# royshil/SfM-Toy-Library

Hardware: AMD Instinct MI355X
Metric: BA LM iterations/sec (200 cams, 100k pts, 1M obs) (higher is better)
Workload: dtype f32 Jacobian blocks and observation coordinates; a lane's own partial sum (<= 8 pair products of a block, ceil(track / 4) point-block products of a point) in f32, every sum across lanes, chunks, points and ranks in f64; residuals, cost, reduced system and solve in f64; 1 GPU; cfg3: 200 cams / 100000 pts / 1000000 obs, shared focal, two-level block-Jacobi PCG, one independent problem per GPU; step=one full LM solve to ceres CONVERGENCE from the resident initial point, linear_solver=two-level block-Jacobi PCG, tolerance 1e-08 anchored to the first LM iteration

## Files before the change

sfm-toy-library_amd/csrc/ba_common.h:

```cpp
#pragma once
#include "ba_kernels.h"
#include "sfmba_device.h"
#include "../../include/sfmba.h"

namespace sfmba {

#define BLK 256

__device__ inline void make_cam_table(const double cam[6], const double* scale6, double* ct) {
    const double w0 = cam[0], w1 = cam[1], w2 = cam[2];
    const double theta2 = w0 * w0 + w1 * w1 + w2 * w2;
    double R[9], K[9];
    double small = 0.0;
    double cq = 1.0 / 12.0;
    if (theta2 > DBL_EPSILON) {
        const double theta = sqrt(theta2);
        double s, c;
        sincos(theta, &s, &c);
        if (theta2 > 1e-8) { const double den = 2.0 * theta * s; cq = fabs(den) > 1e-12 ? 1.0 / theta2 - (1.0 + c) / den : 0.0; }
        const double ti = 1.0 / theta;
        const double k0 = w0 * ti, k1 = w1 * ti, k2 = w2 * ti;
        const double oc = 1.0 - c;
        R[0] = c + k0 * k0 * oc;       R[1] = k0 * k1 * oc - k2 * s;  R[2] = k0 * k2 * oc + k1 * s;
        R[3] = k0 * k1 * oc + k2 * s;  R[4] = c + k1 * k1 * oc;       R[5] = k1 * k2 * oc - k0 * s;
// ... 166 lines not shown
        HalvingReduceT<V, H, OFF / 2, VALU64>::run(v, lane, base, len);
    }
};
template <typename V, int N, bool VALU64>
struct HalvingReduceT<V, N, 0, VALU64> {
    static __device__ __forceinline__ void run(V*, int, int&, int&) {}
};
template <int N, int OFF> using HalvingReduce = HalvingReduceT<double, N, OFF>;

template <typename T>
__device__ __forceinline__ void load_obs(const void* base, int q, double& ox, double& oy) {
    const typename ObsXY<T>::type v = reinterpret_cast<const typename ObsXY<T>::type*>(base)[q];
    ox = (double)v.x; oy = (double)v.y;
}

#ifndef PBK
#define PBK 128
#endif
#define WPB (PBK / 64)

__device__ __forceinline__ void wave_lds_fence() {
    __builtin_amdgcn_fence(__ATOMIC_ACQ_REL, "workgroup");
    __builtin_amdgcn_wave_barrier();
}

#define PB_LPP 4

#define CD_N 48
#define CD_BLK 256
#define CD_OBS (SFMBA_CAM_CHUNK / CD_BLK)
// ... 100 lines not shown
```

sfm-toy-library_amd/csrc/ba_kernels.h:

```cpp
#pragma once
#include <hip/hip_runtime.h>
#include <vector>
#include <stdint.h>

#ifndef SFMBA_CAM_CHUNK
#define SFMBA_CAM_CHUNK 256
#endif

#ifndef SFMBA_PAIR_CHUNK
#define SFMBA_PAIR_CHUNK 512
#endif

namespace sfmba {

enum {
    ACC_TRIAL_COST = 0,
    ACC_MODEL = 1,
    ACC_STEP2 = 2,
    ACC_XNEW2 = 3,
    ACC_BAD_TRIAL = 4,
    ACC_GMAX = 5,
    ACC_BAD_LIN = 6,
    ACC_LIN_COST = 7,
    ACC_COUNT = 8,
// ... 107 lines not shown
    double* pcg_zero;
    int pcg_zero_n;
    double* pcg_bt;
    double* pcg_binv;
    double* pair_partial;
    double* pair_G;
    double* pcg_W;
    int* lm_mailbox;
    double* probe_z;
    double* probe_dpt;
    double shared_weight;
    float* shard_blocks32;
    double* shard_blocks;
    const double* shard_scal;
    const int* shard_row_shift;
};

template <typename T> void launch_cam_setup(hipStream_t s, const DeviceStructure& ds, const DeviceBuffers& db, int which);
void launch_begin(hipStream_t s, const DeviceStructure& ds, const DeviceBuffers& db, const LMState& st, const double* cam_src = nullptr,
                  const double* pts_src = nullptr);
void launch_xnorm(hipStream_t s, const DeviceStructure& ds, const DeviceBuffers& db);
template <typename T> void launch_colnorm(hipStream_t s, const DeviceStructure& ds, const DeviceBuffers& db, int jacobi_scaling, bool clear_udiag = true,
                                         bool points = true, bool finish_xnorm = false, bool with_xnorm = false);
void launch_colnorm_points_only(hipStream_t s, const DeviceStructure& ds, const DeviceBuffers& db, int jacobi, int precision_f32);
void launch_colnorm_cams_only(hipStream_t s, const DeviceStructure& ds, const DeviceBuffers& db, int jacobi, int precision_f32, bool clear_udiag = true);
void launch_colnorm_finish(hipStream_t s, const DeviceStructure& ds, const DeviceBuffers& db, int jacobi);
void launch_iter0(hipStream_t s, const DeviceStructure& ds, const DeviceBuffers& db);

template <typename T> void launch_point_build(hipStream_t s, const DeviceStructure& ds, const DeviceBuffers& db,
                                             int ps_mode = 0 );

template <typename T> void launch_cam_diag(hipStream_t s, const DeviceStructure& ds, const DeviceBuffers& db);

void launch_finalize(hipStream_t s, const DeviceStructure& ds, const DeviceBuffers& db, int pcg);
void launch_cd_fold(hipStream_t s, const DeviceStructure& ds, const DeviceBuffers& db);
void launch_gauge(hipStream_t s, const DeviceStructure& ds, const DeviceBuffers& db);

template <typename T> void launch_schur_pairs(hipStream_t s, const DeviceStructure& ds, const DeviceBuffers& db, int mode);

void launch_cam_update(hipStream_t s, const DeviceStructure& ds, const DeviceBuffers& db);
template <typename T> void launch_point_update(hipStream_t s, const DeviceStructure& ds, const DeviceBuffers& db);
void launch_control(hipStream_t s, const DeviceStructure& ds, const DeviceBuffers& db);

template <typename T> void launch_eval_residuals(hipStream_t s, const DeviceStructure& ds, const DeviceBuffers& db,
                                                 const int* perm, double* res_out, double* cost_out);
template <typename T> void launch_eval_jacobian(hipStream_t s, const DeviceStructure& ds, const DeviceBuffers& db,
                                                const int* obs_pt, const int* perm, double* jc, double* jp, double* jf);
void launch_mirror_scale(hipStream_t s, const DeviceStructure& ds, const DeviceBuffers& db, double* S_full, double* scale_out);

struct ImplicitProduct {
    DeviceStructure ds;
    DeviceBuffers db;
    double* dtab = nullptr;
    double* spt = nullptr;
    double* acc = nullptr;
    double* part = nullptr;
// ... 60 lines not shown
```

sfm-toy-library_amd/csrc/ba_points.hip:

```cpp
#include "ba_common.h"
#include <algorithm>

namespace sfmba {

__device__ __forceinline__ bool chol3_inverse(const double V[6] , double Li[6]) {
    const double i00 = fast_rsq(V[0]);
    const double l10 = V[1] * i00, l20 = V[3] * i00;
    const double d1 = V[2] - l10 * l10;
    const double i11 = fast_rsq(d1);
    const double l21 = (V[4] - l20 * l10) * i11;
    const double d2 = V[5] - l20 * l20 - l21 * l21;
    const double i22 = fast_rsq(d2);
    Li[0] = i00;
    Li[1] = -l10 * i00 * i11;
    Li[2] = i11;
    Li[4] = -l21 * i11 * i22;
    Li[3] = -(l20 * i00 + l21 * Li[1]) * i22;
    Li[5] = i22;
    return (V[0] > 0.0) && (d1 > 0.0) && (d2 > 0.0);
}

template <typename T>
__device__ __forceinline__ void point_finish(const DeviceBuffers& db, const LMState* st, size_t i, int ps_mode, const double (&Xl)[3], double (&V)[6], double (&bp)[3],
                                             double (&Ef)[3], double (&sp)[3], bool store, double& gmax, double& sff, double& rhsf, double& bad) {
// ... 34 lines not shown
    ra.X[0] = Xl[0]; ra.X[1] = Xl[1]; ra.X[2] = Xl[2];
    ra.L[0] = (T)(Li[0] * sp[0]); ra.L[1] = (T)(Li[1] * sp[0]); ra.L[2] = (T)(Li[2] * sp[1]);
    ra.L[3] = (T)(Li[3] * sp[0]); ra.L[4] = (T)(Li[4] * sp[1]); ra.L[5] = (T)(Li[5] * sp[2]);
    if (sizeof(T) == 8) reinterpret_cast<double*>(&ra)[9] = 0.0;
    reinterpret_cast<PtRecA<T>*>(db.PA)[i] = ra;
    PtRecB<T> rb;
    rb.t[0] = (T)t0; rb.t[1] = (T)t1; rb.t[2] = (T)t2;
    rb.yf[0] = (T)y0; rb.yf[1] = (T)y1; rb.yf[2] = (T)y2;
    reinterpret_cast<PtRecB<T>*>(db.PB)[i] = rb;
}

template <typename T>
__global__ __launch_bounds__(PBK) void k_point_build(DeviceStructure ds, DeviceBuffers db, int ps_mode_flags) {
    if ((ps_mode_flags & 4) && (db.st->termination != -1 || db.st->retry != 0)) return;
    const int ps_mode = ps_mode_flags & 3;
    __shared__ double scratch[WPB * 4];
    const LMState* st = db.st;
    const int cur = st->cur;
    const double* tab = db.camtab[cur];
    const double focal = st->focal[cur];
    const T fscale = (T)st->fscale;
    const double* pts = db.pts[cur];
    const int lane = threadIdx.x & 63, w = threadIdx.x >> 6;
    const int gw = blockIdx.x * WPB + w;
    double lin_cost = 0.0, sff = 0.0, rhsf = 0.0, gmax = 0.0, bad = 0.0;
    for (int e = blockIdx.x * blockDim.x + threadIdx.x; e < ds.ncam * 60; e += gridDim.x * blockDim.x) {
        const int j = e / 60, k = e - 60 * j, row0 = 6 * j;
        if (k < 36) db.S[(size_t)(row0 + k / 6) * ds.ld + row0 + k % 6] = 0.0;
        else if (k < 42) db.udiag[row0 + k - 36] = 0.0;
        else if (k < 48) db.bc[row0 + k - 42] = 0.0;
        else if (k < 54) db.rhs[row0 + k - 48] = 0.0;
        else db.S[(size_t)(row0 + k - 54) * ds.ld + ds.d - 1] = 0.0;
    }
    const int sub = lane & (PB_LPP - 1);
    const int slot = gw * (64 / PB_LPP) + (lane / PB_LPP);
    const bool have = slot < ds.npt;
    const int ip = have ? (ds.pt_order ? ds.pt_order[slot] : slot) : 0;
    const size_t i = (size_t)ip;
    const int q0 = have ? ds.pt_ptr[ip] : 0, q1 = have ? ds.pt_ptr[ip + 1] : 0;
    double Xl[3] = { pts[3 * i], pts[3 * i + 1], pts[3 * i + 2] };
    double sp[3] = { 1.0, 1.0, 1.0 };
    if (ps_mode == 0) { sp[0] = db.pscale[3 * i]; sp[1] = db.pscale[3 * i + 1]; sp[2] = db.pscale[3 * i + 2]; }
    T Va[6] = { (T)0, (T)0, (T)0, (T)0, (T)0, (T)0 }, Ea[3] = { (T)0, (T)0, (T)0 };
    double bp[3] = { 0, 0, 0 };
    int q = q0 + sub;
    int j_next = q < q1 ? ds.obs_cam[q] : 0;
    double ox_next = 0.0, oy_next = 0.0;
    if (q < q1) load_obs<T>(ds.obs_xy, q, ox_next, oy_next);
    while (__any(q < q1)) {
        const bool act = q < q1;
        const int j = j_next;
        const double ox = ox_next, oy = oy_next;
        const CamRow ct = { tab + 4 * (size_t)(j), ds.ncam };
        double Rt[12];
#pragma unroll
        for (int e = 0; e < 12; ++e) Rt[e] = ct[CT_R + e];
        q += PB_LPP;
        if (q < q1) { j_next = ds.obs_cam[q]; load_obs<T>(ds.obs_xy, q, ox_next, oy_next); }
        if (act) {
            const Proj pr = project_point(Rt, 0, 9, Xl);
            const double r0 = focal * pr.xp - ox, r1 = focal * pr.yp - oy;
            lin_cost += r0 * r0 + r1 * r1;
            T B[6];
            point_block<T>(Rt, pr, focal, B);
            const T g0 = (T)pr.xp * fscale, g1 = (T)pr.yp * fscale;
            Va[0] += B[0] * B[0] + B[3] * B[3];
            Va[1] += B[1] * B[0] + B[4] * B[3];
            Va[2] += B[1] * B[1] + B[4] * B[4];
            Va[3] += B[2] * B[0] + B[5] * B[3];
            Va[4] += B[2] * B[1] + B[5] * B[4];
            Va[5] += B[2] * B[2] + B[5] * B[5];
#pragma unroll
            for (int c = 0; c < 3; ++c) {
                Ea[c] += B[c] * g0 + B[3 + c] * g1;
                bp[c] += (double)B[c] * r0 + (double)B[3 + c] * r1;
            }
        }
    }
    double V[6], Ef[3];
#pragma unroll
    for (int c = 0; c < 6; ++c) { double v = (double)Va[c]; v = xlane_add<1>(v); v = xlane_add<2>(v); V[c] = v; }
#pragma unroll
    for (int c = 0; c < 3; ++c) {
        double v = (double)Ea[c]; v = xlane_add<1>(v); v = xlane_add<2>(v); Ef[c] = v;
        double u = bp[c]; u = xlane_add<1>(u); u = xlane_add<2>(u); bp[c] = u;
    }
    if (have) point_finish<T>(db, st, i, ps_mode, Xl, V, bp, Ef, sp, sub == 0, gmax, sff, rhsf, bad);
    if (!finite_d(lin_cost)) bad = 1.0;
    const double gm = wave_max(gmax);
    if ((threadIdx.x & 63) == 0 && gm > 0.0) atomic_max_nonneg(slot_ptr(db, ACC_GMAX), gm);
    double sums[4] = { lin_cost, sff, rhsf, bad };
    const double tot = block_sums<4>(sums, scratch);
    if (threadIdx.x < 4) {
        const int which = threadIdx.x == 0 ? ACC_LIN_COST : threadIdx.x == 1 ? ACC_SFF : threadIdx.x == 2 ? ACC_RHSF : ACC_BAD_LIN;
        if (threadIdx.x < 3 || tot != 0.0) atomicAdd(slot_ptr(db, which), tot);
    }
}

template <typename T>
void launch_point_build(hipStream_t s, const DeviceStructure& ds, const DeviceBuffers& db, int ps_mode) {
    const int per_wg = WPB * (64 / PB_LPP);
    hipLaunchKernelGGL(k_point_build<T>, dim3(std::max(1, (ds.npt + per_wg - 1) / per_wg)), dim3(PBK), 0, s, ds, db, ps_mode);
}
template void launch_point_build<float>(hipStream_t, const DeviceStructure&, const DeviceBuffers&, int);
template void launch_point_build<double>(hipStream_t, const DeviceStructure&, const DeviceBuffers&, int);

}
```

sfm-toy-library_amd/csrc/ba_setup.hip:

```cpp
#include "ba_common.h"
#include <algorithm>

namespace sfmba {

__global__ void k_cam_setup(int ncam, const double* __restrict__ cam, const double* __restrict__ cscale, double* __restrict__ camtab) {
    const int j = blockIdx.x * blockDim.x + threadIdx.x;
    if (j >= ncam) return;
    double c6[6], ct[CT_STRIDE];
    for (int e = 0; e < 6; ++e) c6[e] = cam[6 * j + e];
    make_cam_table(c6, cscale + 6 * j, ct);
    for (int e = 0; e < CT_STRIDE; ++e) camtab[cam_tab_index(e, j, ncam)] = ct[e];
}

template <typename T>
void launch_cam_setup(hipStream_t s, const DeviceStructure& ds, const DeviceBuffers& db, int which) {
    hipLaunchKernelGGL(k_cam_setup, dim3((ds.ncam + 63) / 64), dim3(64), 0, s, ds.ncam, db.cam[which], db.cscale, db.camtab[which]);
}
template void launch_cam_setup<float>(hipStream_t, const DeviceStructure&, const DeviceBuffers&, int);
template void launch_cam_setup<double>(hipStream_t, const DeviceStructure&, const DeviceBuffers&, int);

__global__ void k_begin(LMState st, DeviceStructure ds, DeviceBuffers db, const double* __restrict__ cam_src, const double* __restrict__ pts_src) {
    const int e = blockIdx.x * blockDim.x + threadIdx.x;
    if (e == 0) { *db.st = st; *db.lin_info = 0; *db.fin_counter = 0; }
    if (e < 6 * ds.ncam) db.cscale[e] = 1.0;
// ... 36 lines not shown
    hipLaunchKernelGGL(k_xnorm, dim3(blocks), dim3(BLK), 0, s, ds, db);
}

template <typename T>
__global__ __launch_bounds__(BLK) void k_colnorm_points(DeviceStructure ds, DeviceBuffers db, int jacobi) {
    const int i = blockIdx.x * blockDim.x + threadIdx.x;
    if (i >= ds.npt) return;
    const int cur = db.st->cur;
    const double* tab = db.camtab[cur];
    const double focal = db.st->focal[cur];
    const double X[3] = { db.pts[cur][3 * i], db.pts[cur][3 * i + 1], db.pts[cur][3 * i + 2] };
    double n0 = 0, n1 = 0, n2 = 0;
    if (jacobi) {
        for (int q = ds.pt_ptr[i]; q < ds.pt_ptr[i + 1]; ++q) {
            const CamRow ct = { tab + 4 * (size_t)(ds.obs_cam[q]), ds.ncam };
            const Proj pr = project_point(ct, CT_R, CT_T, X);
            T B[6];
            point_block<T>(ct, pr, focal, B);
            n0 += (double)B[0] * (double)B[0] + (double)B[3] * (double)B[3];
            n1 += (double)B[1] * (double)B[1] + (double)B[4] * (double)B[4];
            n2 += (double)B[2] * (double)B[2] + (double)B[5] * (double)B[5];
        }
        db.pscale[3 * i] = 1.0 / (1.0 + sqrt(n0));
        db.pscale[3 * i + 1] = 1.0 / (1.0 + sqrt(n1));
        db.pscale[3 * i + 2] = 1.0 / (1.0 + sqrt(n2));
    } else {
        db.pscale[3 * i] = db.pscale[3 * i + 1] = db.pscale[3 * i + 2] = 1.0;
    }
}

template <typename T>
__global__ __launch_bounds__(BLK) void k_colnorm_cams(DeviceStructure ds, DeviceBuffers db, int with_xnorm) {
    __shared__ double scratch[(BLK / 64) * 8];
    const int4 ch = ds.chunks_coarse[ds.coarse_order[blockIdx.x]];
    const int j = ch.x;
    const int cur = db.st->cur;
// ... 84 lines not shown
```

sfm-toy-library_amd/csrc/ba_step.hip:

```cpp
#include "ba_common.h"
#include <algorithm>

namespace sfmba {

constexpr int CU_LANES = 4;
constexpr int CU_CAMS = BLK / CU_LANES;
static_assert(CU_CAMS == 64, "k_cam_update: the cameras of a workgroup are summed by one wave");

template <int N, int P, typename V, typename At>
__device__ __forceinline__ void store_share(int t, const V (&v)[N], At at) {
    static_assert(N % P == 0, "whole pieces");
    constexpr int NP = N / P;
#pragma unroll
    for (int k0 = 0; k0 < NP; k0 += CU_LANES) {
        V w[P];
#pragma unroll
        for (int r = 0; r < P; ++r) {
            w[r] = v[P * k0 + r];
#pragma unroll
            for (int u = 1; u < CU_LANES; ++u) if (k0 + u < NP) w[r] = (t == u) ? v[P * (k0 + u) + r] : w[r];
        }
        if (k0 + t < NP) {
#pragma unroll
            for (int r = 0; r < P; ++r) *at(P * (k0 + t) + r) = w[r];
// ... 204 lines not shown
        st->message = MSG_MIN_RADIUS;
    }
    row.cost = report_cost;
    row.trust_region_radius = st->radius;
    if (it < db.trace_cap) db.trace[it] = row;
    st->lin_info = 0;
    if (db.st_mirror) *db.st_mirror = *st;
    lm_post(db.lm_mailbox, seq, st->termination, st->message, st->iter, cg_iters);
}

__global__ void k_lm_control(DeviceBuffers db) { lm_control_body(db); }

#ifndef SFMBA_TRIAL_POSE_MIN_CAMS
#define SFMBA_TRIAL_POSE_MIN_CAMS 400
#endif
template <typename T>
__global__ __launch_bounds__(PBK, 4) void k_point_update(DeviceStructure ds, DeviceBuffers db) {
    __shared__ double scratch[WPB * 5];
    if (db.cg_gate && !db.cg_force && db.cg_gate[0] == 0) return;
    const LMState* st = db.st;
    const int cur = st->cur, nxt = cur ^ 1;
    const double* tab = db.camtab[cur];
    const double* stab = db.steptab;
    const double focal = st->focal[cur], focal_n = st->focal[nxt];
    const double dfoc = focal - focal_n;
    const int lane = threadIdx.x & 63, w = threadIdx.x >> 6;
    const int gw = blockIdx.x * WPB + w;
    double trial = 0.0, model = 0.0, step2 = 0.0, xn2 = 0.0, bad = 0.0;
    const int sub = lane & (PB_LPP - 1);
    const int slot = gw * (64 / PB_LPP) + (lane / PB_LPP);
// ... 76 lines not shown
#pragma unroll
    for (int c = 0; c < 3; ++c) Xn[c] = pa.X[c] - dX[c];
    if (have && sub == 0) {
#pragma unroll
        for (int c = 0; c < 3; ++c) {
            const double df = pa.X[c] - Xn[c];
            step2 += df * df;
            xn2 += Xn[c] * Xn[c];
            db.pts[nxt][3 * i + c] = Xn[c];
            if (db.probe_dpt) db.probe_dpt[3 * i + c] = dX[c];
        }
        const double zGz = Gd[0] * z0 * z0 + Gd[3] * z1 * z1 + Gd[5] * z2 * z2 + 2.0 * (Gd[1] * z0 * z1 + Gd[2] * z0 * z2 + Gd[4] * z1 * z2);
        model += ur + (z0 * tp[0] + z1 * tp[1] + z2 * tp[2]) - 0.5 * uu - (z0 * zacc[0] + z1 * zacc[1] + z2 * zacc[2]) - 0.5 * zGz;
    }
    const bool pose_from_cam = sizeof(T) == 4 && ds.ncam >= SFMBA_TRIAL_POSE_MIN_CAMS;
    {
        int q = q0 + sub;
        int j_next = q < q1 ? ds.obs_cam[q] : 0;
        double ox_next = 0.0, oy_next = 0.0;
        if (q < q1) load_obs<T>(ds.obs_xy, q, ox_next, oy_next);
        while (__any(q < q1)) {
            const bool act = q < q1;
            const int j = j_next;
            const double ox = ox_next, oy = oy_next;
            double RTn[12];
            if (pose_from_cam) {
                const double2* cp = reinterpret_cast<const double2*>(db.cam[nxt] + 6 * (size_t)j);
                const double2 c0 = cp[0], c1 = cp[1], c2 = cp[2];
                const double cn6[6] = { c0.x, c0.y, c1.x, c1.y, c2.x, c2.y };
                pose_from_params(cn6, RTn);
            } else {
                const CamRow stb = { stab + 4 * (size_t)(j), ds.ncam };
#pragma unroll
                for (int e = 0; e < 12; ++e) RTn[e] = stb[ST_RN + e];
            }
            q += PB_LPP;
            if (q < q1) { j_next = ds.obs_cam[q]; load_obs<T>(ds.obs_xy, q, ox_next, oy_next); }
            if (act) {
                const Proj pn = project_point(RTn, 0, 9, Xn);
                const double n0 = focal_n * pn.xp - ox, n1 = focal_n * pn.yp - oy;
                if (!finite_d(n0) || !finite_d(n1)) bad = 1.0;
                trial += n0 * n0 + n1 * n1;
            }
        }
    }
    double sums[5] = { trial, model, step2, xn2, bad };
    const double tot = block_sums<5>(sums, scratch);
    if (threadIdx.x < 5) {
        const int which = threadIdx.x == 0 ? ACC_TRIAL_COST : threadIdx.x == 1 ? ACC_MODEL : threadIdx.x == 2 ? ACC_STEP2 : threadIdx.x == 3 ? ACC_XNEW2 : ACC_BAD_TRIAL;
        if (threadIdx.x < 4 || tot != 0.0) atomicAdd(slot_ptr(db, which), tot);
    }
}

void launch_cam_update(hipStream_t s, const DeviceStructure& ds, const DeviceBuffers& db) {
    hipLaunchKernelGGL(k_cam_update, dim3((ds.ncam + CU_CAMS - 1) / CU_CAMS), dim3(BLK), 0, s, ds, db);
}

template <typename T>
void launch_point_update(hipStream_t s, const DeviceStructure& ds, const DeviceBuffers& db) {
    const int per_wg = WPB * (64 / PB_LPP);
    hipLaunchKernelGGL(k_point_update<T>, dim3(std::max(1, (ds.npt + per_wg - 1) / per_wg)), dim3(PBK), 0, s, ds, db);
}
template void launch_point_update<float>(hipStream_t, const DeviceStructure&, const DeviceBuffers&);
template void launch_point_update<double>(hipStream_t, const DeviceStructure&, const DeviceBuffers&);

void launch_control(hipStream_t s, const DeviceStructure& ds, const DeviceBuffers& db) {
    (void)ds;
    hipLaunchKernelGGL(k_lm_control, dim3(1), dim3(64), 0, s, db);
}

}
```

sfm-toy-library_amd/csrc/lm_loop.h:

```cpp
#pragma once
#include "problem.h"

namespace sfmba {
void init_state(sfmba_problem* p, LMState& st, const sfmba_options& o);
int upload_state(sfmba_problem* p, const LMState& st);
int download_state(sfmba_problem* p);
int ensure_trace(sfmba_problem* p, int rows);
int probe_arm(sfmba_problem* p);
void probe_note(sfmba_problem* p, int family, int f32_matrix, int coarse_vectors, int cholesky_fallback);
void probe_note_solver(sfmba_problem* p, bool pcg, int cholesky_fallback);
int run_solve(sfmba_problem* p, const sfmba_options& o, sfmba_summary* summary, sfmba_iteration* trace, int trace_cap, int* trace_len);

int solve_matrix_free(sfmba_problem* p, const sfmba_options& o, sfmba_summary* summary, sfmba_iteration* trace, int trace_cap, int* trace_len);

void launch_unit_cscale(sfmba_problem* p);

template <typename T>
void launch_back_substitution(hipStream_t s, const DeviceStructure& ds, const DeviceStructure& ds_points, const DeviceBuffers& dbu, Profiler* prof) {
    DeviceBuffers b = dbu;
    if (sizeof(T) == 8) b.pu32 = nullptr;
    { ProfScope ps(prof, KID_CAM_UPDATE, s); launch_cam_update(s, ds, b); }
    { ProfScope ps(prof, KID_POINT_UPDATE, s); launch_point_update<T>(s, ds_points, b); }
}

// ... 1 lines not shown
void launch_linearise_setup(sfmba_problem* p, int jacobi, bool begun = false) {
    if (begun) {
        const bool fold = jacobi && p->ds.nchunk_coarse > 0;
        if (!fold) launch_xnorm(p->stream, p->ds, p->db);
        launch_colnorm<T>(p->stream, p->ds, p->db, jacobi, false, false, true, fold);
        return;
    }
    launch_unit_cscale(p);
    launch_cam_setup<T>(p->stream, p->ds, p->db, p->cur);
    launch_xnorm(p->stream, p->ds, p->db);
    launch_iter0(p->stream, p->ds, p->db);
    launch_colnorm<T>(p->stream, p->ds, p->db, jacobi);
}

template <typename T>
void launch_partial_linearisation(sfmba_problem* p, int ps_mode, bool point_pass_done = false) {
    if (!point_pass_done) launch_point_build<T>(p->stream, p->ds, p->db, ps_mode);
    launch_cam_diag<T>(p->stream, p->ds, p->db);
    launch_schur_pairs<T>(p->stream, p->ds, p->db, 2);
    launch_schur_pairs<T>(p->stream, p->ds, p->db, 0);
}

struct LinearPlan {
    bool cg;
    bool exact;
    double tol;
    int max_iters;
    bool anchored;
    int anchor(bool first_solve) const { return anchored ? (first_solve ? 1 : 2) : 0; }
};
LinearPlan linear_plan(const sfmba_options& o, int d, bool always_cg, bool cap_auto_iters);
inline void keep_both_triangles(sfmba_problem* p) { p->solver.symmetric = false; p->db.pcg_upper_only = 0; p->db.pcg_zero = nullptr; p->db.pcg_zero_n = 0; }
// ... 9 lines not shown
```

sfm-toy-library_amd/csrc/lm_solve.hip:

```cpp
#include "lm_loop.h"
#include "sfmba_device.h"
#include <dlfcn.h>
#include <mutex>
#include <thread>

namespace sfmba {
namespace {
const char* message_text(int id) {
    static const char* const text[] = { "", "Gradient tolerance reached.", "Parameter tolerance reached.", "Function tolerance reached.",
        "Minimum trust region radius reached.", "Number of consecutive invalid steps more than max_num_consecutive_invalid_steps.",
        "Initial residual and Jacobian evaluation failed.", "Residual and Jacobian evaluation failed.", "Maximum number of iterations reached.",
        "Maximum solver time reached." };
    static_assert(MSG_NONE == 0 && MSG_MAX_TIME == 9, "message ids index the table");
    return id >= 0 && id <= MSG_MAX_TIME ? text[id] : "";
}

int wait_mailbox(volatile int* word, int want, hipStream_t stream) {
    const double t0 = now_seconds();
    unsigned spins = 0;
    double next_query = 2e-3;
    for (;;) {
        if (*word >= want) { __sync_synchronize(); return 0; }
        ++spins;
        if ((spins & 63u) != 0u) { __builtin_ia32_pause(); continue; }
// ... 202 lines not shown
    int host_iter = 0;
    bool state_mirrored = false;
    bool first_linearisation = true;
    bool first_linear_solve = true;
    const bool f32_matrix = option_switch(o.pcg_f32_matrix, true);
    const bool coarse_cg = option_switch(o.pcg_coarse_space, true);
    const bool segments_cg = coarse_cg && (dense_pcg_segments_applicable(&p->solver) || dense_pcg_segments_streaming_applicable(&p->solver)) &&
                             option_switch(o.pcg_coarse_space == 2 ? 1 : o.pcg_coarse_space == 1 ? -1 : 0, p->block_fill < 0.5 && p->block_band >= 0.9);
    const bool symmetric_cg = option_switch(o.pcg_symmetric, true) && !p->deterministic &&
                              !(segments_cg && dense_pcg_segments_streaming_applicable(&p->solver));
    const LinearPlan plan = linear_plan(o, p->ds.d, false, true);
    const bool pcg_mode = plan.cg, exact_pcg = plan.exact;
    const int nblk64 = p->ds.ld / 64;
    const int cg_break_even = std::max(30, (nblk64 <= 40 ? 33 : 20) * nblk64 / 10);
    int launched_controls = 0;
    const bool speculate = option_switch(o.early_linearise, true) && !p->prof.on;
    bool build_enqueued = false;
    std::vector<int> lin_hist;
    int cholesky_fallbacks = 0;
    bool auto_prefers_cholesky = false;
    if (exact_pcg && p->block_fill < 0.5 && p->block_band >= 0.9 && !(segments_cg && dense_pcg_segments_streaming_applicable(&p->solver))) auto_prefers_cholesky = true;
    p->h_lm_mail[0] = 0; p->h_lm_mail[1] = -1;
    for (;;) {
        if (o.max_seconds > 0.0 && now_seconds() - t0 >= o.max_seconds) { term = SFMBA_NO_CONVERGENCE; msg = MSG_MAX_TIME; break; }
        if (host_iter >= o.max_iters) {
            term = SFMBA_NO_CONVERGENCE; msg = MSG_MAX_ITERS;
            if (host_iter == 0) {
                launch_partial_linearisation<T>(p, o.jacobi_scaling ? 1 : 2);
                launch_finalize(p->stream, p->ds, p->db, 0);
                HIP_TRY(hipGetLastError());
// ... 10 lines not shown
            if (dense_pcg_ensure_workspace(&p->solver)) return fail(SFMBA_ERR_ALLOC, "PCG workspace allocation failed");
            p->db.pcg_F = p->solver.Sfull;
            p->db.pcg_W = coarse_cg ? p->solver.W : nullptr;
            p->db.pcg_F32 = (p->precision == SFMBA_PRECISION_F32J && f32_matrix) ? dense_pcg_want_f32(&p->solver) : nullptr;
            p->solver.use_f32 = p->db.pcg_F32 != nullptr;
            p->solver.symmetric = symmetric_cg && dense_pcg_symmetric_applicable(&p->solver);
            p->db.pcg_upper_only = p->solver.symmetric ? 1 : 0;
            p->db.pcg_zero = p->solver.symmetric ? p->solver.sym_zero : nullptr;
            p->db.pcg_zero_n = p->solver.symmetric ? (int)p->solver.sym_zero_n : 0;
        }
        RoctxRange rx_iter(p->roctx, "sfmba LM iteration");
        {
        RoctxRange rx(p->roctx, "linearise: point_build + cam_diag");
        if (!build_enqueued) {
            ProfScope ps(prof, KID_POINT_BUILD, p->stream);
            launch_point_build<T>(p->stream, p->ds, p->db, first_linearisation ? (o.jacobi_scaling ? 1 : 2) : 0);
        }
        build_enqueued = false;
        first_linearisation = false;
        { ProfScope ps(prof, KID_CAM_DIAG, p->stream); launch_cam_diag<T>(p->stream, p->ds, p->db); }
        launch_schur_pairs<T>(p->stream, p->ds, p->db, 2);
        }
        RoctxRange rx_reduce(p->roctx, "reduce: finalize + schur_pairs (reduced camera system)");
        if (pcg) {
            { ProfScope ps(prof, KID_FINALIZE, p->stream); launch_finalize(p->stream, p->ds, p->db, 1); }
            { ProfScope ps(prof, KID_SCHUR_PAIRS, p->stream); launch_schur_pairs<T>(p->stream, p->ds, p->db, 1); }
        } else {
            { ProfScope ps(prof, KID_SCHUR_PAIRS, p->stream); launch_schur_pairs<T>(p->stream, p->ds, p->db, 0); }
            { ProfScope ps(prof, KID_FINALIZE, p->stream); launch_finalize(p->stream, p->ds, p->db, 0); }
        }
        rx_reduce.end();
        DeviceBuffers dbu = p->db;
        if (sizeof(T) == 4) dbu.pu32 = p->d_pu32;
        bool pcg_gated = false;
        bool fell_back = false;
        RoctxRange rx_solve(p->roctx, pcg ? "solve: two-level CG on the reduced system" : "solve: Cholesky of the reduced system");
        if (pcg) {
            pcg_gated = true;
            const int it = dense_pcg_solve(p->stream, &p->solver, p->db.S, p->db.rhs, plan.tol, plan.max_iters, p->d_info, prof,
                                           { .finish = false, .hist_key = host_iter, .pretransformed = true, .anchor = plan.anchor(first_linear_solve), .no_wait = true,
                                             .coarse = coarse_cg, .segments = segments_cg });
            first_linear_solve = false;
            if (it < 0) return fail(SFMBA_ERR_ALLOC, "PCG workspace allocation failed");
            dbu.pcg_vec = p->solver.vec; dbu.pcg_linv = p->solver.binv; dbu.pcg_flags = p->solver.flags;
            dbu.cg_gate = pcg_gated ? p->solver.flags : nullptr;
            dbu.cg_force = 0;
        } else {
            dense_cholesky_solve(p->stream, &p->solver, p->db.S, p->db.rhs, p->d_info, prof);
            lin_hist.push_back(0);
        }
        rx_solve.end();
        RoctxRange rx_update(p->roctx, "update: cam_update + point_update + lm_control (and the wait for its verdict)");
        bool lm_done = false;
        while (!lm_done) {
            launch_back_substitution<T>(p->stream, p->ds, p->ds, dbu, prof);
            probe_note_solver(p, pcg && !fell_back, fell_back ? 1 : 0);
            { ProfScope ps(prof, KID_CONTROL, p->stream); launch_control(p->stream, p->ds, dbu); }
            { ProfScope ps(prof, KID_EMPTY, p->stream); }
            ++launched_controls;
            if ((rc = launches_ok())) return rc;
            if (speculate && host_iter + 2 <= o.max_iters) {
                ProfScope ps(prof, KID_POINT_BUILD, p->stream);
                launch_point_build<T>(p->stream, p->ds, p->db, 4);
                build_enqueued = true;
            }
            if ((rc = await_control(p, launched_controls, "LM iteration did not complete on the device: ", "stream drained without the control kernel's post"))) return rc;
            volatile int* mb = p->h_lm_mail;
            if (mb[1] == -2) {
                if (dense_pcg_more(p->stream, &p->solver, 8, prof) == 0) {
                    if (exact_pcg) {
                        { ProfScope ps(prof, KID_SCHUR_PAIRS, p->stream); launch_schur_pairs<T>(p->stream, p->ds, p->db, 0); }
                        dense_cholesky_solve(p->stream, &p->solver, p->db.S, p->db.rhs, p->d_info, prof);
                        dbu.pcg_vec = nullptr; dbu.pcg_linv = nullptr; dbu.pcg_flags = nullptr; dbu.cg_gate = nullptr;
                        pcg_gated = false;
                        fell_back = true;
                        ++cholesky_fallbacks;
                    } else {
                        dbu.cg_force = 1;
// ... 13 lines not shown
                if (p->probe_on) p->probe.cg_iters = it;
                sum.linear_iters += it;
                lin_hist.push_back(it);
            }
        }
        if (term != -1) break;
        if (o.verbose) {
            rc = download_state(p);
            if (rc) return rc;
            std::fprintf(stderr, "[sfmba] it %3d cost %.12e |g|inf %.3e radius %.3e term %d\n", p->h_state->iter, p->h_state->cost,
                         p->h_state->gmax, p->h_state->radius, p->h_state->termination);
        }
    }
    if (host_iter > 0 && term == SFMBA_NO_CONVERGENCE && (msg == MSG_MAX_ITERS || msg == MSG_MAX_TIME) && state_mirrored &&
        p->h_state->termination == -1 && p->h_state->x_is_new) {
        launch_partial_linearisation<T>(p, 0, build_enqueued);
        launch_finalize(p->stream, p->ds, p->db, 0);
        if ((rc = launches_ok())) return rc;
        HIP_TRY(hipStreamSynchronize(p->stream));
        if ((rc = download_state(p))) return rc;
        if (p->h_state->termination == SFMBA_FAILURE) { term = p->h_state->termination; msg = p->h_state->message; }
    }
    if (!state_mirrored || p->prof.on) {
        HIP_TRY(hipStreamSynchronize(p->stream));
        rc = download_state(p);
        if (rc) return rc;
    }
    if (p->prof.on) p->prof.collect();
    fill_summary(p, sum, t0);
    set_termination(sum, term, msg);
    sum.cholesky_fallbacks = cholesky_fallbacks;
// ... 16 lines not shown
```

sfm-toy-library_amd/csrc/problem.h:

```cpp
#pragma once
#include "../../include/sfmba.h"
#include "ba_kernels.h"
#include "dense_solver.h"
#include "dist_cg.h"
#include "device_arena.h"
#include "profiler.h"
#include <algorithm>
#include <chrono>
#include <cstdio>
#include <cstdlib>
#include <cstring>
#include <string>
#include <vector>

struct sfmba_problem {
    int device = 0;
    int precision = SFMBA_PRECISION_F64;
    hipStream_t stream = nullptr;
    int n_cam_full = 0, n_pt_full = 0;
    int64_t n_obs = 0;
    std::vector<int> acam_id, apt_id;
    std::vector<int> h_pt_cnt, h_cam_cnt;
    std::vector<int> cam_slot, pt_slot;
    bool sharded = false;
    sfmba::DeviceStructure ds = {};
    sfmba::DeviceBuffers db = {};
    sfmba::DenseSolver solver;
    sfmba::DeviceArena arena;
    sfmba::HostKit kit;
    int *d_pt_ptr = nullptr, *d_obs_cam = nullptr, *d_cam_ptr = nullptr, *d_cam_obs = nullptr, *d_cam_obs_pt = nullptr;
    int *d_obs_pt = nullptr, *d_perm = nullptr;
    void* d_obs_xy = nullptr;
    int4* d_chunks = nullptr, *d_chunks_coarse = nullptr, *d_pwg_desc = nullptr;
    float* d_pu32 = nullptr;
    int2* d_pwg_chunk = nullptr; int* d_multi_slots = nullptr; int* d_build_counters = nullptr; int* d_pt_order = nullptr;
    int *d_chunk_order = nullptr, *d_coarse_order = nullptr;
    double block_fill = 1.0;
    double block_band = 0.0;
    int* d_blk_ptr = nullptr;
    unsigned* d_blk_mask = nullptr;
    int* d_cam_chunk_ptr = nullptr;
    bool deterministic = false;
    bool roctx = false;
    bool cam_identity = false, pt_identity = false;
    bool reset_pending = false;
    int2 *d_blk_cams = nullptr, *d_pwg_blocks = nullptr, *d_dup_blocks = nullptr;
    int* d_pair_pt = nullptr;
    void* d_cam_obs_xy = nullptr;
    double* d_facc = nullptr;
// ... 107 lines not shown
```

sfm-toy-library_amd/csrc/problem_build.hip:

```cpp
#include "problem.h"
#include "sfmba_device.h"
#include <atomic>
#include <cmath>
#include <condition_variable>
#include <functional>
#include <mutex>
#include <thread>

using namespace sfmba;

thread_local DeviceArena* sfmba::t_arena = nullptr;

namespace {
struct BuildStopwatch {
    const char* tag;
    const bool on = std::getenv("SFMBA_BUILD_TIMING") != nullptr;
    double t = now_seconds();
    void mark(const char* what) { if (on) { const double n = now_seconds(); std::fprintf(stderr, "[sfmba %s] %-18s %.3f ms\n", tag, what, 1e3 * (n - t)); t = now_seconds(); } }
};

constexpr int PARALLEL_FOR_MIN = 200000;
template <typename F>
void parallel_for(int n, F fn) {
    unsigned nt = n >= PARALLEL_FOR_MIN ? std::min(8u, std::max(1u, std::thread::hardware_concurrency())) : 1u;
// ... 382 lines not shown
    db = DeviceBuffers{};
    for (int b = 0; b < 2; ++b) {
        HIP_TRY(dev_alloc(&db.cam[b], (size_t)6 * ncam));
        HIP_TRY(dev_alloc(&db.pts[b], (size_t)3 * npt_alloc));
        HIP_TRY(dev_alloc(&db.camtab[b], (size_t)CT_STRIDE * ncam));
    }
    HIP_TRY(dev_alloc(&db.steptab, (size_t)ST_STRIDE * ncam));
    HIP_TRY(dev_alloc(&p->d_pu32, (size_t)20 * std::max(ncam, 1)));
    HIP_TRY(dev_alloc(&db.cscale, (size_t)6 * ncam));
    HIP_TRY(dev_alloc(&db.pscale, (size_t)3 * npt));
    db.PA = p->arena.alloc(std::max<size_t>(npt_alloc, 1) * (f32 ? sizeof(PtRecA<float>) : sizeof(PtRecA<double>)));
    db.PB = p->arena.alloc(std::max<size_t>(npt_alloc, 1) * (f32 ? sizeof(PtRecB<float>) : sizeof(PtRecB<double>)));
    if (!db.PA || !db.PB) return fail(SFMBA_ERR_ALLOC, "device allocation failed");
    HIP_TRY(dev_alloc(&db.pt_t, (size_t)3 * npt));
    HIP_TRY(dev_alloc(&db.pt_M, (size_t)6 * npt));
    const size_t sys_len = (size_t)ds.ld * ds.ld + 3 * (size_t)ds.ld + SFMBA_SHARD_SCALARS;
    HIP_TRY(dev_alloc(&p->d_sys, sys_len));
    p->d_red = nullptr;
    if (no_pairs) {
        p->shard_blocks_off = (shard_diag_len(ds) + 63) / 64 * 64;
        HIP_TRY(dev_alloc(&p->d_red, (size_t)p->shard_blocks_off));
        p->dcg = DistCg(); p->dcg_last_f32 = -1;
        p->imp_dtab = p->imp_spt = p->imp_acc = p->imp_part = nullptr;
    }
    if (sharded) {
        const size_t tri = (size_t)ds.ld * (ds.ld + 1) / 2 + 3 * (size_t)ds.ld + SFMBA_SHARD_SCALARS;
        std::vector<int> rows; long long chunk = 0;
        dcg_partition(ncam, p->shard_world, &rows, &chunk);
        p->shard_blocks_off = (shard_diag_len(ds) + 63) / 64 * 64;
        const size_t dist = (size_t)p->shard_blocks_off + (size_t)p->shard_world * (size_t)chunk * 36;
// ... 247 lines not shown
```

Measured before the change: 4829 LM iterations/s.

## Carry point Hessian sums from trial evaluation into the next linearisation

During the trial-cost sweep, the point update kernel now also accumulates each point's 3x3 Hessian block, its camera-coupling term and its gradient. It writes them to a double-buffered per-point sums array. When the step is accepted, the next point_build reads these stored sums and skips its own pass over the observations, and it also skips adding the linearised cost, which equals the trial cost already counted. Floating-point contraction is pinned in a shared projection helper so the two paths agree numerically. The trade is extra arithmetic and stores in every trial sweep, including rejected ones, plus two extra per-point buffers.

```diff
diff --git a/sfm-toy-library_amd/csrc/ba_common.h b/sfm-toy-library_amd/csrc/ba_common.h
--- a/sfm-toy-library_amd/csrc/ba_common.h
+++ b/sfm-toy-library_amd/csrc/ba_common.h
@@ -204,6 +204,72 @@
     ox = (double)v.x; oy = (double)v.y;
 }
 
+__device__ __forceinline__ float fma_t(float a, float b, float c) { return __builtin_fmaf(a, b, c); }
+__device__ __forceinline__ double fma_t(double a, double b, double c) { return __builtin_fma(a, b, c); }
+template <typename T, bool BLOCK>
+__device__ __forceinline__ void point_proj_pinned(const double (&Rt)[12], const double (&X)[3], double focal, double ox, double oy, double& r0, double& r1, T (&B)[6], T& xp, T& yp) {
+#pragma clang fp contract(off)
+    const double px = fma_t(Rt[2], X[2], fma_t(Rt[0], X[0], Rt[1] * X[1])) + Rt[9];
+    const double py = fma_t(Rt[5], X[2], fma_t(Rt[4], X[1], Rt[3] * X[0])) + Rt[10];
+    const double pz = fma_t(Rt[8], X[2], fma_t(Rt[6], X[0], Rt[7] * X[1])) + Rt[11];
+    const double iz = fast_rcp(pz);
+    const double xpd = px * iz, ypd = py * iz;
+    r0 = fma_t(focal, xpd, -ox); r1 = fma_t(focal, ypd, -oy);
+    if constexpr (BLOCK) {
+        const T fz = (T)(focal * iz);
+        xp = (T)xpd; yp = (T)ypd;
+#pragma unroll
+        for (int c = 0; c < 3; ++c) {
+            const T a0 = (T)Rt[c], a1 = (T)Rt[3 + c], a2 = (T)Rt[6 + c];
+            B[c] = fz * fma_t(-xp, a2, a0);
+            B[3 + c] = fz * fma_t(-yp, a2, a1);
+        }
+    }
+}
+__device__ __forceinline__ double sq2_pinned(double a, double b) {
+#pragma clang fp contract(off)
+    return fma_t(a, a, b * b);
+}
+template <typename T, bool ACCUMULATE>
+__device__ __forceinline__ double point_obs_pinned(const double (&Rt)[12], const double (&X)[3], double focal, T fscale, double ox, double oy, double& r0, double& r1,
+                                                   T (&Va)[6], T (&Ea)[3], double (&bp)[3]) {
+#pragma clang fp contract(off)
+    T B[6], xp, yp;
+    point_proj_pinned<T, ACCUMULATE>(Rt, X, focal, ox, oy, r0, r1, B, xp, yp);
+    if constexpr (ACCUMULATE) {
+        const T g0 = xp * fscale, g1 = yp * fscale;
+        Va[0] += fma_t(B[3], B[3], B[0] * B[0]);
+        Va[1] += fma_t(B[1], B[0], B[4] * B[3]);
+        Va[2] += fma_t(B[1], B[1], B[4] * B[4]);
+        Va[3] += fma_t(B[2], B[0], B[5] * B[3]);
+        Va[4] += fma_t(B[5], B[4], B[2] * B[1]);
+        Va[5] += fma_t(B[2], B[2], B[5] * B[5]);
+        Ea[0] += B[0] * g0 + B[3] * g1;
+        Ea[1] += fma_t(B[1], g0, B[4] * g1);
+        Ea[2] += fma_t(B[2], g0, B[5] * g1);
+#pragma unroll
+        for (int c = 0; c < 3; ++c) bp[c] += fma_t((double)B[c], r0, (double)B[3 + c] * r1);
+    }
+    return fma_t(r0, r0, r1 * r1);
+}
+
+template <typename T>
+__device__ __forceinline__ void quad_point_sums(const T (&Va)[6], const T (&Ea)[3], double (&bp)[3], double (&V)[6], double (&Ef)[3]) {
+#pragma unroll
+    for (int c = 0; c < 6; ++c) { double v = (double)Va[c]; v = xlane_add<1>(v); v = xlane_add<2>(v); V[c] = v; }
+#pragma unroll
+    for (int c = 0; c < 3; ++c) {
+        double v = (double)Ea[c]; v = xlane_add<1>(v); v = xlane_add<2>(v); Ef[c] = v;
+        double u = bp[c]; u = xlane_add<1>(u); u = xlane_add<2>(u); bp[c] = u;
+    }
+}
+
+__device__ __forceinline__ void store_point_sums(double* dst, const double (&V)[6], const double (&Ef)[3], const double (&bp)[3]) {
+    double2* d2 = reinterpret_cast<double2*>(dst);
+    d2[0] = make_double2(V[0], V[1]); d2[1] = make_double2(V[2], V[3]); d2[2] = make_double2(V[4], V[5]);
+    d2[3] = make_double2(Ef[0], Ef[1]); d2[4] = make_double2(Ef[2], bp[0]); d2[5] = make_double2(bp[1], bp[2]);
+}
+
 #ifndef PBK
 #define PBK 128
 #endif
diff --git a/sfm-toy-library_amd/csrc/ba_kernels.h b/sfm-toy-library_amd/csrc/ba_kernels.h
--- a/sfm-toy-library_amd/csrc/ba_kernels.h
+++ b/sfm-toy-library_amd/csrc/ba_kernels.h
@@ -145,7 +145,9 @@
     double* shard_blocks;
     const double* shard_scal;
     const int* shard_row_shift;
-};
+    double* ptsums[2];
+};
+constexpr int PTSUMS_N = 12;
 
 template <typename T> void launch_cam_setup(hipStream_t s, const DeviceStructure& ds, const DeviceBuffers& db, int which);
 void launch_begin(hipStream_t s, const DeviceStructure& ds, const DeviceBuffers& db, const LMState& st, const double* cam_src = nullptr,
@@ -171,6 +173,7 @@
 
 void launch_cam_update(hipStream_t s, const DeviceStructure& ds, const DeviceBuffers& db);
 template <typename T> void launch_point_update(hipStream_t s, const DeviceStructure& ds, const DeviceBuffers& db);
+template <typename T> bool point_update_carries_sums(const DeviceStructure& ds);
 void launch_control(hipStream_t s, const DeviceStructure& ds, const DeviceBuffers& db);
 
 template <typename T> void launch_eval_residuals(hipStream_t s, const DeviceStructure& ds, const DeviceBuffers& db,
diff --git a/sfm-toy-library_amd/csrc/ba_points.hip b/sfm-toy-library_amd/csrc/ba_points.hip
--- a/sfm-toy-library_amd/csrc/ba_points.hip
+++ b/sfm-toy-library_amd/csrc/ba_points.hip
@@ -72,6 +72,7 @@
 __global__ __launch_bounds__(PBK) void k_point_build(DeviceStructure ds, DeviceBuffers db, int ps_mode_flags) {
     if ((ps_mode_flags & 4) && (db.st->termination != -1 || db.st->retry != 0)) return;
     const int ps_mode = ps_mode_flags & 3;
+    const bool from_sums = (ps_mode_flags & 8) != 0;
     __shared__ double scratch[WPB * 4];
     const LMState* st = db.st;
     const int cur = st->cur;
@@ -99,49 +100,37 @@
     double Xl[3] = { pts[3 * i], pts[3 * i + 1], pts[3 * i + 2] };
     double sp[3] = { 1.0, 1.0, 1.0 };
     if (ps_mode == 0) { sp[0] = db.pscale[3 * i]; sp[1] = db.pscale[3 * i + 1]; sp[2] = db.pscale[3 * i + 2]; }
-    T Va[6] = { (T)0, (T)0, (T)0, (T)0, (T)0, (T)0 }, Ea[3] = { (T)0, (T)0, (T)0 };
-    double bp[3] = { 0, 0, 0 };
-    int q = q0 + sub;
-    int j_next = q < q1 ? ds.obs_cam[q] : 0;
-    double ox_next = 0.0, oy_next = 0.0;
-    if (q < q1) load_obs<T>(ds.obs_xy, q, ox_next, oy_next);
-    while (__any(q < q1)) {
-        const bool act = q < q1;
-        const int j = j_next;
-        const double ox = ox_next, oy = oy_next;
-        const CamRow ct = { tab + 4 * (size_t)(j), ds.ncam };
-        double Rt[12];
+    double V[6], Ef[3], bp[3] = { 0, 0, 0 };
+    double* const sums_cur = cur ? db.ptsums[1] : db.ptsums[0];
+    if (from_sums) {
+        const double2* sp2 = reinterpret_cast<const double2*>(sums_cur + PTSUMS_N * (size_t)(have ? slot : 0));
+        const double2 s0 = sp2[0], s1 = sp2[1], s2 = sp2[2], s3 = sp2[3], s4 = sp2[4], s5 = sp2[5];
+        V[0] = s0.x; V[1] = s0.y; V[2] = s1.x; V[3] = s1.y; V[4] = s2.x; V[5] = s2.y;
+        Ef[0] = s3.x; Ef[1] = s3.y; Ef[2] = s4.x; bp[0] = s4.y; bp[1] = s5.x; bp[2] = s5.y;
+    } else {
+        T Va[6] = { (T)0, (T)0, (T)0, (T)0, (T)0, (T)0 }, Ea[3] = { (T)0, (T)0, (T)0 };
+        int q = q0 + sub;
+        int j_next = q < q1 ? ds.obs_cam[q] : 0;
+        const typename ObsXY<T>::type* const obs_xy = reinterpret_cast<const typename ObsXY<T>::type*>(ds.obs_xy);
+        typename ObsXY<T>::type o_next = {};
+        if (q < q1) o_next = obs_xy[q];
+        while (__any(q < q1)) {
+            const bool act = q < q1;
+            const int j = j_next;
+            const double ox = (double)o_next.x, oy = (double)o_next.y;
+            const CamRow ct = { tab + 4 * (size_t)(j), ds.ncam };
+            double Rt[12];
 #pragma unroll
-        for (int e = 0; e < 12; ++e) Rt[e] = ct[CT_R + e];
-        q += PB_LPP;
-        if (q < q1) { j_next = ds.obs_cam[q]; load_obs<T>(ds.obs_xy, q, ox_next, oy_next); }
-        if (act) {
-            const Proj pr = project_point(Rt, 0, 9, Xl);
-            const double r0 = focal * pr.xp - ox, r1 = focal * pr.yp - oy;
-            lin_cost += r0 * r0 + r1 * r1;
-            T B[6];
-            point_block<T>(Rt, pr, focal, B);
-            const T g0 = (T)pr.xp * fscale, g1 = (T)pr.yp * fscale;
-            Va[0] += B[0] * B[0] + B[3] * B[3];
-            Va[1] += B[1] * B[0] + B[4] * B[3];
-            Va[2] += B[1] * B[1] + B[4] * B[4];
-            Va[3] += B[2] * B[0] + B[5] * B[3];
-            Va[4] += B[2] * B[1] + B[5] * B[4];
-            Va[5] += B[2] * B[2] + B[5] * B[5];
-#pragma unroll
-            for (int c = 0; c < 3; ++c) {
-                Ea[c] += B[c] * g0 + B[3 + c] * g1;
-                bp[c] += (double)B[c] * r0 + (double)B[3 + c] * r1;
+            for (int e = 0; e < 12; ++e) Rt[e] = ct[CT_R + e];
+            q += PB_LPP;
+            if (q < q1) { j_next = ds.obs_cam[q]; o_next = obs_xy[q]; }
+            if (act) {
+                double r0, r1;
+                lin_cost += point_obs_pinned<T, true>(Rt, Xl, focal, fscale, ox, oy, r0, r1, Va, Ea, bp);
             }
         }
-    }
-    double V[6], Ef[3];
-#pragma unroll
-    for (int c = 0; c < 6; ++c) { double v = (double)Va[c]; v = xlane_add<1>(v); v = xlane_add<2>(v); V[c] = v; }
-#pragma unroll
-    for (int c = 0; c < 3; ++c) {
-        double v = (double)Ea[c]; v = xlane_add<1>(v); v = xlane_add<2>(v); Ef[c] = v;
-        double u = bp[c]; u = xlane_add<1>(u); u = xlane_add<2>(u); bp[c] = u;
+        quad_point_sums<T>(Va, Ea, bp, V, Ef);
+        if (sums_cur && have && sub == 0) store_point_sums(sums_cur + PTSUMS_N * (size_t)slot, V, Ef, bp);
     }
     if (have) point_finish<T>(db, st, i, ps_mode, Xl, V, bp, Ef, sp, sub == 0, gmax, sff, rhsf, bad);
     if (!finite_d(lin_cost)) bad = 1.0;
@@ -151,14 +140,16 @@
     const double tot = block_sums<4>(sums, scratch);
     if (threadIdx.x < 4) {
         const int which = threadIdx.x == 0 ? ACC_LIN_COST : threadIdx.x == 1 ? ACC_SFF : threadIdx.x == 2 ? ACC_RHSF : ACC_BAD_LIN;
-        if (threadIdx.x < 3 || tot != 0.0) atomicAdd(slot_ptr(db, which), tot);
+        if ((threadIdx.x < 3 || tot != 0.0) && !(from_sums && threadIdx.x == 0)) atomicAdd(slot_ptr(db, which), tot);
     }
 }
 
 template <typename T>
 void launch_point_build(hipStream_t s, const DeviceStructure& ds, const DeviceBuffers& db, int ps_mode) {
     const int per_wg = WPB * (64 / PB_LPP);
-    hipLaunchKernelGGL(k_point_build<T>, dim3(std::max(1, (ds.npt + per_wg - 1) / per_wg)), dim3(PBK), 0, s, ds, db, ps_mode);
+    const dim3 grid(std::max(1, (ds.npt + per_wg - 1) / per_wg));
+    const bool from_sums = (ps_mode & 8) && (ps_mode & 3) == 0 && db.ptsums[0] && db.ptsums[1];
+    hipLaunchKernelGGL(k_point_build<T>, grid, dim3(PBK), 0, s, ds, db, from_sums ? ps_mode : ps_mode & ~8);
 }
 template void launch_point_build<float>(hipStream_t, const DeviceStructure&, const DeviceBuffers&, int);
 template void launch_point_build<double>(hipStream_t, const DeviceStructure&, const DeviceBuffers&, int);
diff --git a/sfm-toy-library_amd/csrc/ba_setup.hip b/sfm-toy-library_amd/csrc/ba_setup.hip
--- a/sfm-toy-library_amd/csrc/ba_setup.hip
+++ b/sfm-toy-library_amd/csrc/ba_setup.hip
@@ -74,12 +74,14 @@
     if (jacobi) {
         for (int q = ds.pt_ptr[i]; q < ds.pt_ptr[i + 1]; ++q) {
             const CamRow ct = { tab + 4 * (size_t)(ds.obs_cam[q]), ds.ncam };
-            const Proj pr = project_point(ct, CT_R, CT_T, X);
-            T B[6];
-            point_block<T>(ct, pr, focal, B);
-            n0 += (double)B[0] * (double)B[0] + (double)B[3] * (double)B[3];
-            n1 += (double)B[1] * (double)B[1] + (double)B[4] * (double)B[4];
-            n2 += (double)B[2] * (double)B[2] + (double)B[5] * (double)B[5];
+            double Rt[12], r0, r1;
+#pragma unroll
+            for (int e = 0; e < 12; ++e) Rt[e] = ct[CT_R + e];
+            T B[6], xp, yp;
+            point_proj_pinned<T, true>(Rt, X, focal, 0.0, 0.0, r0, r1, B, xp, yp);
+            n0 += sq2_pinned((double)B[3], (double)B[0]);
+            n1 += sq2_pinned((double)B[1], (double)B[4]);
+            n2 += sq2_pinned((double)B[2], (double)B[5]);
         }
         db.pscale[3 * i] = 1.0 / (1.0 + sqrt(n0));
         db.pscale[3 * i + 1] = 1.0 / (1.0 + sqrt(n1));
diff --git a/sfm-toy-library_amd/csrc/ba_step.hip b/sfm-toy-library_amd/csrc/ba_step.hip
--- a/sfm-toy-library_amd/csrc/ba_step.hip
+++ b/sfm-toy-library_amd/csrc/ba_step.hip
@@ -1,5 +1,6 @@
 #include "ba_common.h"
 #include <algorithm>
+#include <type_traits>
 
 namespace sfmba {
 
@@ -242,6 +243,10 @@
 #ifndef SFMBA_TRIAL_POSE_MIN_CAMS
 #define SFMBA_TRIAL_POSE_MIN_CAMS 400
 #endif
+#ifndef SFMBA_POINT_SUMS_F64
+#define SFMBA_POINT_SUMS_F64 0
+#endif
+#define SFMBA_POINT_SUMS_CARRY(T) (sizeof(T) == 4 || SFMBA_POINT_SUMS_F64)
 template <typename T>
 __global__ __launch_bounds__(PBK, 4) void k_point_update(DeviceStructure ds, DeviceBuffers db) {
     __shared__ double scratch[WPB * 5];
@@ -348,7 +353,13 @@
         model += ur + (z0 * tp[0] + z1 * tp[1] + z2 * tp[2]) - 0.5 * uu - (z0 * zacc[0] + z1 * zacc[1] + z2 * zacc[2]) - 0.5 * zGz;
     }
     const bool pose_from_cam = sizeof(T) == 4 && ds.ncam >= SFMBA_TRIAL_POSE_MIN_CAMS;
-    {
+    constexpr bool CARRY = SFMBA_POINT_SUMS_CARRY(T);
+    double* const sums_nxt = CARRY && !pose_from_cam ? (cur ? db.ptsums[0] : db.ptsums[1]) : nullptr;
+    auto trial_sweep = [&](auto from_cam, auto with_sums) {
+        constexpr bool FROM_CAM = decltype(from_cam)::value, WITH_SUMS = decltype(with_sums)::value;
+        const T fscale = (T)st->fscale;
+        T Va[6] = { (T)0, (T)0, (T)0, (T)0, (T)0, (T)0 }, Ea[3] = { (T)0, (T)0, (T)0 };
+        double bp[3] = { 0, 0, 0 };
         int q = q0 + sub;
         int j_next = q < q1 ? ds.obs_cam[q] : 0;
         double ox_next = 0.0, oy_next = 0.0;
@@ -358,7 +369,7 @@
             const int j = j_next;
             const double ox = ox_next, oy = oy_next;
             double RTn[12];
-            if (pose_from_cam) {
+            if constexpr (FROM_CAM) {
                 const double2* cp = reinterpret_cast<const double2*>(db.cam[nxt] + 6 * (size_t)j);
                 const double2 c0 = cp[0], c1 = cp[1], c2 = cp[2];
                 const double cn6[6] = { c0.x, c0.y, c1.x, c1.y, c2.x, c2.y };
@@ -371,13 +382,27 @@
             q += PB_LPP;
             if (q < q1) { j_next = ds.obs_cam[q]; load_obs<T>(ds.obs_xy, q, ox_next, oy_next); }
             if (act) {
-                const Proj pn = project_point(RTn, 0, 9, Xn);
-                const double n0 = focal_n * pn.xp - ox, n1 = focal_n * pn.yp - oy;
+                double n0, n1, n2;
+                if constexpr (FROM_CAM) {
+                    const Proj pn = project_point(RTn, 0, 9, Xn);
+                    n0 = focal_n * pn.xp - ox; n1 = focal_n * pn.yp - oy;
+                    n2 = n0 * n0 + n1 * n1;
+                } else {
+                    n2 = point_obs_pinned<T, WITH_SUMS>(RTn, Xn, focal_n, fscale, ox, oy, n0, n1, Va, Ea, bp);
+                }
                 if (!finite_d(n0) || !finite_d(n1)) bad = 1.0;
-                trial += n0 * n0 + n1 * n1;
-            }
-        }
-    }
+                trial += n2;
+            }
+        }
+        if constexpr (WITH_SUMS) {
+            double V[6], Ef[3];
+            quad_point_sums<T>(Va, Ea, bp, V, Ef);
+            if (have && sub == 0) store_point_sums(sums_nxt + PTSUMS_N * (size_t)slot, V, Ef, bp);
+        }
+    };
+    if (pose_from_cam) trial_sweep(std::true_type{}, std::false_type{});
+    else if (CARRY && sums_nxt) trial_sweep(std::false_type{}, std::integral_constant<bool, CARRY>{});
+    else trial_sweep(std::false_type{}, std::false_type{});
     double sums[5] = { trial, model, step2, xn2, bad };
     const double tot = block_sums<5>(sums, scratch);
     if (threadIdx.x < 5) {
@@ -398,6 +423,13 @@
 template void launch_point_update<float>(hipStream_t, const DeviceStructure&, const DeviceBuffers&);
 template void launch_point_update<double>(hipStream_t, const DeviceStructure&, const DeviceBuffers&);
 
+template <typename T>
+bool point_update_carries_sums(const DeviceStructure& ds) {
+    return SFMBA_POINT_SUMS_CARRY(T) && !(sizeof(T) == 4 && ds.ncam >= SFMBA_TRIAL_POSE_MIN_CAMS);
+}
+template bool point_update_carries_sums<float>(const DeviceStructure&);
+template bool point_update_carries_sums<double>(const DeviceStructure&);
+
 void launch_control(hipStream_t s, const DeviceStructure& ds, const DeviceBuffers& db) {
     (void)ds;
     hipLaunchKernelGGL(k_lm_control, dim3(1), dim3(64), 0, s, db);
diff --git a/sfm-toy-library_amd/csrc/lm_loop.h b/sfm-toy-library_amd/csrc/lm_loop.h
--- a/sfm-toy-library_amd/csrc/lm_loop.h
+++ b/sfm-toy-library_amd/csrc/lm_loop.h
@@ -39,8 +39,12 @@
 }
 
 template <typename T>
-void launch_partial_linearisation(sfmba_problem* p, int ps_mode, bool point_pass_done = false) {
-    if (!point_pass_done) launch_point_build<T>(p->stream, p->ds, p->db, ps_mode);
+void launch_partial_linearisation(sfmba_problem* p, int ps_mode, bool point_pass_done = false, double* const* ptsums = nullptr) {
+    if (!point_pass_done) {
+        DeviceBuffers b = p->db;
+        if (ptsums) { b.ptsums[0] = ptsums[0]; b.ptsums[1] = ptsums[1]; }
+        launch_point_build<T>(p->stream, p->ds, b, ps_mode);
+    }
     launch_cam_diag<T>(p->stream, p->ds, p->db);
     launch_schur_pairs<T>(p->stream, p->ds, p->db, 2);
     launch_schur_pairs<T>(p->stream, p->ds, p->db, 0);
diff --git a/sfm-toy-library_amd/csrc/lm_solve.hip b/sfm-toy-library_amd/csrc/lm_solve.hip
--- a/sfm-toy-library_amd/csrc/lm_solve.hip
+++ b/sfm-toy-library_amd/csrc/lm_solve.hip
@@ -240,6 +240,9 @@
     const int nblk64 = p->ds.ld / 64;
     const int cg_break_even = std::max(30, (nblk64 <= 40 ? 33 : 20) * nblk64 / 10);
     int launched_controls = 0;
+    const bool carry = p->d_ptsums[0] && p->d_ptsums[1] && point_update_carries_sums<T>(p->ds);
+    auto with_sums = [&](DeviceBuffers b) { if (carry) { b.ptsums[0] = p->d_ptsums[0]; b.ptsums[1] = p->d_ptsums[1]; } return b; };
+    const int from_sums = carry ? 8 : 0;
     const bool speculate = option_switch(o.early_linearise, true) && !p->prof.on;
     bool build_enqueued = false;
     std::vector<int> lin_hist;
@@ -280,7 +283,7 @@
         RoctxRange rx(p->roctx, "linearise: point_build + cam_diag");
         if (!build_enqueued) {
             ProfScope ps(prof, KID_POINT_BUILD, p->stream);
-            launch_point_build<T>(p->stream, p->ds, p->db, first_linearisation ? (o.jacobi_scaling ? 1 : 2) : 0);
+            launch_point_build<T>(p->stream, p->ds, with_sums(p->db), first_linearisation ? (o.jacobi_scaling ? 1 : 2) : from_sums);
         }
         build_enqueued = false;
         first_linearisation = false;
@@ -296,7 +299,7 @@
             { ProfScope ps(prof, KID_FINALIZE, p->stream); launch_finalize(p->stream, p->ds, p->db, 0); }
         }
         rx_reduce.end();
-        DeviceBuffers dbu = p->db;
+        DeviceBuffers dbu = with_sums(p->db);
         if (sizeof(T) == 4) dbu.pu32 = p->d_pu32;
         bool pcg_gated = false;
         bool fell_back = false;
@@ -327,7 +330,7 @@
             if ((rc = launches_ok())) return rc;
             if (speculate && host_iter + 2 <= o.max_iters) {
                 ProfScope ps(prof, KID_POINT_BUILD, p->stream);
-                launch_point_build<T>(p->stream, p->ds, p->db, 4);
+                launch_point_build<T>(p->stream, p->ds, with_sums(p->db), 4 | from_sums);
                 build_enqueued = true;
             }
             if ((rc = await_control(p, launched_controls, "LM iteration did not complete on the device: ", "stream drained without the control kernel's post"))) return rc;
@@ -371,7 +374,7 @@
     }
     if (host_iter > 0 && term == SFMBA_NO_CONVERGENCE && (msg == MSG_MAX_ITERS || msg == MSG_MAX_TIME) && state_mirrored &&
         p->h_state->termination == -1 && p->h_state->x_is_new) {
-        launch_partial_linearisation<T>(p, 0, build_enqueued);
+        launch_partial_linearisation<T>(p, from_sums, build_enqueued, carry ? p->d_ptsums : nullptr);
         launch_finalize(p->stream, p->ds, p->db, 0);
         if ((rc = launches_ok())) return rc;
         HIP_TRY(hipStreamSynchronize(p->stream));
diff --git a/sfm-toy-library_amd/csrc/problem.h b/sfm-toy-library_amd/csrc/problem.h
--- a/sfm-toy-library_amd/csrc/problem.h
+++ b/sfm-toy-library_amd/csrc/problem.h
@@ -33,6 +33,7 @@
     void* d_obs_xy = nullptr;
     int4* d_chunks = nullptr, *d_chunks_coarse = nullptr, *d_pwg_desc = nullptr;
     float* d_pu32 = nullptr;
+    double* d_ptsums[2] = { nullptr, nullptr };
     int2* d_pwg_chunk = nullptr; int* d_multi_slots = nullptr; int* d_build_counters = nullptr; int* d_pt_order = nullptr;
     int *d_chunk_order = nullptr, *d_coarse_order = nullptr;
     double block_fill = 1.0;
diff --git a/sfm-toy-library_amd/csrc/problem_build.hip b/sfm-toy-library_amd/csrc/problem_build.hip
--- a/sfm-toy-library_amd/csrc/problem_build.hip
+++ b/sfm-toy-library_amd/csrc/problem_build.hip
@@ -420,6 +420,12 @@
     if (!db.PA || !db.PB) return fail(SFMBA_ERR_ALLOC, "device allocation failed");
     HIP_TRY(dev_alloc(&db.pt_t, (size_t)3 * npt));
     HIP_TRY(dev_alloc(&db.pt_M, (size_t)6 * npt));
+    p->d_ptsums[0] = p->d_ptsums[1] = nullptr;
+    {
+        const char* e = std::getenv("SFMBA_POINT_SUMS");
+        if (!(e && std::strcmp(e, "rebuild") == 0) && !no_pairs && !sharded)
+            for (int b = 0; b < 2; ++b) HIP_TRY(dev_alloc(&p->d_ptsums[b], (size_t)PTSUMS_N * std::max(npt, 1)));
+    }
     const size_t sys_len = (size_t)ds.ld * ds.ld + 3 * (size_t)ds.ld + SFMBA_SHARD_SCALARS;
     HIP_TRY(dev_alloc(&p->d_sys, sys_len));
     p->d_red = nullptr;
```

Result: faster. 4881 LM iterations/s, median of 6 (+1.1%).
